# QueensGambit/CrazyAra

Measured on AMD Instinct MI355X. Metric: nn_evals_per_sec, higher is better.
Workload: dtype f16x3; 1 GPU; crazyhouse RISEv2 19-block (34x8x8 planes -> 5184 policy + value), batch=256, inputs resident in HBM, random-init seeded weights; batch=256, parallelism=replicas x1, precision=float16x3

## Files before the change

crazyara_amd/csrc/nn/kernels.h:

```cpp
#pragma once
#include <hip/hip_runtime.h>
#include <cstdint>

namespace cra {

typedef _Float16 half_t;

constexpr int kSquares = 64;

inline int64_t packed_weight_elems(int cout_pad, int k_total) { return int64_t(cout_pad) * k_total; }

struct ConvArgs {
    const void* x;
    const void* wpk;
    const void* wpk_lo;
    const float* bias;
    const void* resid;
    void* out;
    int batch;
    int cin;
    int cout_pad;
    int cout_real;
    int cout_ld;
    int ks;
// ... 237 lines not shown
    int batch, C, cv, fc;
    float* dbg;
    int lds_pad;
    int variant;
};
template <typename T> void prepare_value_head(const ValueHeadArgs& a);
size_t value_head_lds_bytes(const ValueHeadArgs& a);
template <typename T> void launch_value_head(const ValueHeadArgs& a, hipStream_t s);

struct HeadsSmallArgs {
    ConvArgs conv;
    ValueHeadArgs vh;
};
bool heads_small_fits(const ConvArgs& c, const ValueHeadArgs& v);
void launch_heads_small(const HeadsSmallArgs& a, hipStream_t s);

struct ValueFinalArgs {
    const void* in;
    int n;
    const float* w;
    float b[4];
    int wdlp;
    float* value;
    float* aux;
    int batch;
};
template <typename T> void launch_value_final(const ValueFinalArgs& a, hipStream_t s);

void launch_gather_probs(const float* probs, int nb_policy, const uint16_t* idx, const uint32_t* cnt, int stride, int n_slots, float* out,
                         const float* value_dev, float* value_out, int batch, const float* aux_dev, float* aux_out, hipStream_t s);
// ... 23 lines not shown
```

crazyara_amd/csrc/nn/precision.cpp:

```cpp
#include <cstdlib>
#include <stdexcept>

#include "rise_net.h"

namespace cra {

namespace {
constexpr bool kX3ValueHeadOneLaunch = true;
}

RiseNet::DevSwitches::DevSwitches() {
    if (const char* e = getenv("CRA_X3_CONV_DEV")) conv_dev = atoi(e);
    device_graph = getenv("CRA_DEVICE_GRAPH") != nullptr;
    lane_graph = getenv("CRA_LANE_GRAPH") != nullptr;
    lane_no_graph = getenv("CRA_LANE_NO_GRAPH") != nullptr;
    predict_copy = getenv("CRA_PREDICT_COPY") != nullptr;
    predict_zero_copy = getenv("CRA_PREDICT_ZERO_COPY") != nullptr;
    if (const char* e = getenv("CRA_LANE_LAUNCHES")) lane_launches = e[0];
    lane_sync = getenv("CRA_LANE_SYNC") != nullptr;
    if (const char* e = getenv("CRA_X3_TOWER")) x3_symmetric = e[0] == 's';
    if (const char* e = getenv("CRA_X3_SPLIT_DEV")) x3_split_dev = atoi(e);
    no_small_path = getenv("CRA_NO_SMALL_PATH") != nullptr;
    if (const char* e = getenv("CRA_SMALL_BATCH_CONV_SPLIT")) small_conv_split = atoi(e);
    tower_trace = getenv("CRA_TOWER_TRACE") != nullptr;
    x3_value_one_launch = kX3ValueHeadOneLaunch;
    if (const char* e = getenv("CRA_X3_VALUE_HEAD")) x3_value_one_launch = e[0] == 'o';
    value_head_debug = getenv("CRA_VALUE_HEAD_DEBUG") != nullptr;
    if (const char* e = getenv("CRA_VALUE_HEAD_LDS_PAD")) value_head_lds_pad = atoi(e);
    if (const char* e = getenv("CRA_VALUE_HEAD_VARIANT")) value_head_variant = atoi(e);
    x3_no_head_chain = getenv("CRA_X3_NO_HEAD_CHAIN") != nullptr;
    x3_no_tail = getenv("CRA_X3_NO_TAIL") != nullptr;
    small_batch_heads_apart = getenv("CRA_SMALL_BATCH_HEADS_APART") != nullptr;
}

Precision parse_precision(const std::string& precision) {
    Precision v;
    std::string prec = precision;
    auto strip = [&](const std::string& tag) {
        if (prec.size() <= tag.size() || prec.compare(prec.size() - tag.size(), tag.size(), tag) != 0) return false;
        prec.resize(prec.size() - tag.size());
        return true;
    };
    if (strip("-3k")) v.one_launch = false;
    if (strip("-8w")) v.thin_waves = true;
    if (strip("-1wg")) v.board_split = false;
// ... 31 lines not shown
```

crazyara_amd/csrc/nn/rise_net.h:

```cpp
#pragma once
#include <hip/hip_runtime.h>
#include <memory>
#include <string>
#include <utility>
#include <vector>

#include "board_net.h"
#include "netfile.h"

namespace cra {

uint8_t float_to_e4m3(float v);
uint8_t float_to_e5m2(float v);

struct Precision {
    enum class Mode { Float32, Float16, Float16x3, Float16p8, Fp8, Int8 };
    Mode mode = Mode::Float16;
    bool fused = true;
    bool tower = true;
    bool one_launch = true;
    bool thin_waves = false;
    bool board_split = true;
    bool wblock = false;
    bool wnet = false;
// ... 91 lines not shown
        bool lane_no_graph = false;
        bool predict_copy = false;
        bool predict_zero_copy = false;
        char lane_launches = 0;
        bool lane_sync = false;
        bool x3_symmetric = false;
        int x3_split_dev = 0;
        bool no_small_path = false;
        int small_conv_split = 2;
        bool tower_trace = false;
        bool x3_value_one_launch;
        bool value_head_debug = false;
        int value_head_lds_pad = -1;
        int value_head_variant = 0;
        bool x3_no_head_chain = false;
        bool x3_no_tail = false;
        bool small_batch_heads_apart = false;
        DevSwitches();
    } dev_;
    float* value_head_dbg_ = nullptr;

    std::string model_file_path_;
    Precision prec_;
    std::vector<std::pair<float, float>> int8_calib_;
    static constexpr int kBoardSplitMaxBatch = 64;
    std::unique_ptr<RiseNet> small_;
    bool owns_stream_ = true;
    int stream_slot_ = -1;
    std::string precision_arg_;
    int cu_count_ = 256;
// ... 14 lines not shown
```

crazyara_amd/csrc/nn/rise_net.hip:

```cpp
#include "rise_net.h"

#include <cmath>
#include <cstdio>
#include <cstring>
#include <fstream>
#include <algorithm>

#include "net_streams.h"
#include "onnx_import.h"
#include "rise_net_impl.h"
#include "../chess/planes_host.h"

namespace cra {

RiseNet::RiseNet(const std::string& model_path, int device_id, int batch_size, const std::string& precision, const RiseNet* parent)
    : BoardNet(device_id), impl_(new Impl) {
    if (batch_size <= 0) throw std::invalid_argument("batch size must be positive");
    precision_arg_ = precision;
    prec_ = parse_precision(precision);
    design_.batch = batch_size;

    std::string dir, file;
    auto ends_with = [&](const char* ext) { const size_t n = strlen(ext); return model_path.size() > n && model_path.compare(model_path.size() - n, n, ext) == 0; };
    if (ends_with(".cranet") || ends_with(".onnx")) {
// ... 60 lines not shown
    const int B = n > 0 ? n : design_.batch;
    const Op& op = im.ops[i];
    auto boards = [&](ConvArgs c) {
        if (n > 0 && c.batch == design_.batch && !c.out_rows_f32) c.batch = n;
        return c;
    };
    const float* planes = io ? io->planes : d_planes_;
    float* value = io ? io->value : d_value_;
    float* probs = io ? io->probs : d_probs_;
    float* aux = (io && d_aux_) ? (io->aux ? io->aux : d_aux_) : d_aux_;
    switch (op.kind) {
        case OpKind::PlanesToAct:
            launch_planes_to_act<T>(op.x == d_planes_ ? planes : static_cast<const float*>(op.x), static_cast<T*>(op.y), B, op.C, im.cin_pad, s);
            break;
        case OpKind::Conv:
            if (prec_.x3() && dev_.conv_dev >= 0) {
                ConvArgs c = boards(op.conv);
                c.dev = dev_.conv_dev;
                if (op.from_planes) c.planes = planes;
                if (op.fused_softmax) { c.softmax_out = probs; if (!keep_logits_) c.out = nullptr; }
                launch_conv_gemm_x3(c, s);
            } else if (prec_.x3() && op.from_planes) {
                ConvArgs c = boards(op.conv);
                c.planes = planes;
                launch_conv_gemm_x3(c, s);
            } else if (prec_.x3() && op.fused_softmax) {
                ConvArgs c = boards(op.conv);
                c.softmax_out = probs;
                if (!keep_logits_) c.out = nullptr;
                launch_conv_gemm_x3(c, s);
            } else if (prec_.x3()) launch_conv_gemm_x3(boards(op.conv), s);
// ... 623 lines not shown
```

crazyara_amd/csrc/nn/rise_net_build.hip:

```cpp
#include <algorithm>
#include <cmath>
#include <cstring>
#include <type_traits>

#include "../chess/planes_host.h"
#include "pack.h"
#include "rise_net_impl.h"

namespace cra {

namespace {
enum class Family {
    Tower,
    X3Tower,
    X3Split,
    Fused,
    WBlock,
    WSplit,
    Layers,
    Transformer,
    WNtb
};
struct BlockPlan {
    Family family;
// ... 48 lines not shown
    void add_se(Op op, bool consumer_fused);
    void stem();
    void dense_tower();
    void dense_layer_blocks();
    void bottleneck_blocks();
    void transformer_block(size_t i);
    void transformer_block_x3w(const NtbFold& n);
    void flush_tower();
    void flush_x3_run();
    void wsplit_finish();
    void one_launch_head();
    void policy_head();
    void softmax();
    void value_head();
    void merge_heads_small();
    void merge_forward();
};

template <typename T> void RiseNet::Builder<T>::read_model() {
    B = net.design_.batch;
    cin = int(nf.num("nb_input_channels"));
    C = int(nf.num("channels", 256));
    const int cop_init = int(nf.num("channels_operating_init"));
    const int cexp = int(nf.num("channel_expansion"));
    cv = int(nf.num("channels_value_head", 8));
    fc = int(nf.num("value_fc_size", 256));
    cp = int(nf.num("channels_policy_head"));
    wdl = nf.num("use_wdl") != 0 && nf.num("use_plys_to_end") != 0;
    std::vector<std::string> kernels = nf.list("kernels");
    se_types = nf.list("se_types");
// ... 784 lines not shown
    im.ops.push_back(op);
}

template <typename T> void RiseNet::Builder<T>::merge_heads_small() {
    std::vector<Op>& ops = im.ops;
    if (x3_split && ops.size() >= 2 && ops.back().kind == OpKind::ValueHead && ops[ops.size() - 2].kind == OpKind::Conv &&
        ops[ops.size() - 2].fused_softmax && heads_small_fits(ops[ops.size() - 2].conv, ops.back().vh) && !dev.small_batch_heads_apart) {
        Op vh = ops.back();
        ops.pop_back();
        Op& op = ops.back();
        op.kind = OpKind::HeadsSmall;
        op.vh = vh.vh;
    }
}

template <typename T> void RiseNet::Builder<T>::merge_forward() {
    std::vector<Op>& ops = im.ops;
    if (prec.one_launch && ops.size() == 3 && ops[0].kind == OpKind::Stem && ops[1].kind == OpKind::Tower && ops[2].kind == OpKind::Head &&
        ops[1].tw.gate_in == nullptr && ops[1].tw.pool_out == nullptr) {
        Op op;
        op.kind = OpKind::Forward;
        op.st = ops[0].st;
        op.tw = ops[1].tw;
        op.hd = ops[2].hd;
        ops.assign(1, op);
        init_forward_kernel_attributes();
    }
}

template <typename T> void RiseNet::build(const NetFile& nf) {
// ... 6 lines not shown
    if (prec_.wnet && b.wblock_ops == 0 && b.wntb_ops == 0)
        throw std::runtime_error("`-wnet` runs the mobile-bottleneck and transformer blocks of 128 / 192 / 224-channel nets in one launch each: no block of this model qualifies (" +
                                 std::to_string(b.C) + " channels, " + (b.dense_blocks ? "dense residual blocks" : "mobile-bottleneck blocks") +
                                 "); use the precision without the suffix");
    if (prec_.wblock && !prec_.wnet && b.wblock_ops == 0)
        throw std::runtime_error("`-wblock` runs the mobile-bottleneck blocks of 128 / 192 / 224-channel nets in one launch each: no block of this model qualifies (" +
                                 std::to_string(b.C) + " channels, " + (b.dense_blocks ? "dense residual blocks" : "mobile-bottleneck blocks") +
                                 "); use the precision without the suffix");
    if (b.head_ok) {
        b.one_launch_head();
    } else {
        b.policy_head();
        b.softmax();
        b.value_head();
        b.merge_heads_small();
    }
    init_block_kernel_attributes<T>();
    init_x3_kernel_attributes();
    init_x3_wblock_kernel_attributes();
    init_x3_wsplit_kernel_attributes();
    init_x3_wntb_kernel_attributes();
    init_tower_kernel_attributes();
    init_restower_kernel_attributes();
    init_head_kernel_attributes();
    b.merge_forward();
    design_.flops_per_position = 2.0 * b.macs;
    launches_ = int(impl_->ops.size());
}

template void RiseNet::build<half_t>(const NetFile& nf);
template void RiseNet::build<float>(const NetFile& nf);

}
// ... 1 lines not shown
```

crazyara_amd/csrc/nn/rise_net_impl.h:

```cpp
#pragma once
#include <stdexcept>
#include <string>
#include <utility>
#include <vector>

#include "kernels.h"
#include "rise_net.h"

namespace cra {

#define HIP_CHECK(expr)                                                                                      \
    do {                                                                                                     \
        hipError_t _e = (expr);                                                                              \
        if (_e != hipSuccess)                                                                                \
            throw std::runtime_error(std::string("HIP error ") + hipGetErrorString(_e) + " at " #expr);      \
    } while (0)

enum class OpKind { PlanesToAct, Conv, Depthwise, SE, ValueHead, Softmax, Block, ValueFinal, SEGate, Tower, Head, Stem, ResTower, Forward, TowerX3, BlockX3Split, X3SplitFinish, HeadsSmall, Attention, BlockX3W, NtbX3W, BlockX3WSplit, X3WSplitFinish };

struct Op {
    OpKind kind;
    ConvArgs conv{};
    bool from_planes = false;
    bool fused_softmax = false;
    const void* x = nullptr;
    void* y = nullptr;
    const float *w0 = nullptr, *w1 = nullptr, *b0 = nullptr;
    int C = 0, ks = 0, se_kind = 0;
    ValueHeadArgs vh{};
    BlockArgs blk{};
    NtbArgs ntb{};
    ValueFinalArgs vf{};
    TowerArgs tw{};
    HeadArgs hd{};
    ResTowerArgs rt{};
    StemArgs st{};
    X3TowerArgs tx{};
    X3SplitArgs xs{};
// ... 44 lines not shown
```

crazyara_amd/csrc/nn/x3.hip:

```cpp
#include "kernels.h"
#include "device_utils.h"
#include "value_head_body.h"
#include "x3_device.h"

#include <algorithm>
#include <cstdlib>
#include <stdexcept>
#include <type_traits>

#ifndef X3_SGB_VALU
#define X3_SGB_VALU 10
#endif

namespace cra {

namespace {

typedef int i32x4_x3 __attribute__((ext_vector_type(4)));
typedef int i32x8_x3 __attribute__((ext_vector_type(8)));
__device__ __forceinline__ uint32_t x3_high_bytes(uint32_t p01, uint32_t p23) {
    return __builtin_amdgcn_perm(p23, p01, 0x07050301u);
}
__device__ __forceinline__ void split4_b8(const float (&v)[4], half4& hi, uint32_t& h8, uint32_t& l8) {
    uint32_t h[2], l[2];
// ... 9 lines not shown
    else asm volatile("" : "+v"(c) : "v"(a), "v"(b));
}
__device__ __forceinline__ i32x8_x3 x3_cat(const half8& lo16, const half8& hi16) {
    return __builtin_shufflevector(__builtin_bit_cast(i32x4_x3, lo16), __builtin_bit_cast(i32x4_x3, hi16), 0, 1, 2, 3, 4, 5, 6, 7);
}

__device__ __forceinline__ float fmac_shr1(float acc, float x, float w) { return fmaf(w, dpp_mov<DPP_ROW_SHR1>(x), acc); }
__device__ __forceinline__ float fmac_shl1(float acc, float x, float w) { return fmaf(w, dpp_mov<DPP_ROW_SHL1>(x), acc); }

__device__ __forceinline__ void mma_x3(const half8& ah, const half8& al, const half8& bh, const half8& bl, f32x4& c) {
    c = __builtin_amdgcn_mfma_f32_16x16x32_f16(al, bh, c, 0, 0, 0);
    c = __builtin_amdgcn_mfma_f32_16x16x32_f16(ah, bl, c, 0, 0, 0);
    c = __builtin_amdgcn_mfma_f32_16x16x32_f16(ah, bh, c, 0, 0, 0);
}

constexpr int X3_KC = 128;
constexpr int X3_ROWP = X3_KC + 8;

}

template <int MT, int NW>
__device__ __forceinline__ void conv_x3_finish(const ConvArgs& a, f32x4 (&acc)[MT][4], const bool (&active)[MT], char* smem, int b, int co_tile0, float acc_scale) {
    constexpr int NTHR = 64 * NW;
    const int tid = threadIdx.x;
    const int wave = tid >> 6, lane = tid & 63;
    const int l15 = lane & 15, lg = lane >> 4;
    if (a.softmax_out) __syncthreads();
#pragma unroll
    for (int m = 0; m < MT; ++m) {
        if (!active[m]) continue;
        const int co0 = (co_tile0 + m) * 16 + lg * 4;
        float bs[4];
#pragma unroll
        for (int r = 0; r < 4; ++r) bs[r] = a.bias[co0 + r];
#pragma unroll
        for (int t = 0; t < 4; ++t) {
            const int sq = t * 16 + l15;
            float v[4];
#pragma unroll
            for (int r = 0; r < 4; ++r) v[r] = fmaf(acc[m][t][r], acc_scale, bs[r]);
            if (a.relu == 2) {
#pragma unroll
                for (int r = 0; r < 4; ++r) v[r] = fmaxf(v[r], 0.f);
            }
            if (a.resid) {
                float rv[4];
                load4<float>(reinterpret_cast<const float*>(a.resid) + (size_t(b) * kSquares + sq) * a.cout_ld + co0, rv);
#pragma unroll
                for (int r = 0; r < 4; ++r) v[r] += rv[r];
            }
            if (a.relu == 1) {
#pragma unroll
                for (int r = 0; r < 4; ++r) v[r] = fmaxf(v[r], 0.f);
            }
            if (a.out_policy_f32) {
                float* o = reinterpret_cast<float*>(a.out) + size_t(b) * a.cout_real * kSquares;
                float* lds_logits = reinterpret_cast<float*>(smem);
#pragma unroll
                for (int r = 0; r < 4; ++r)
                    if (co0 + r < a.cout_real) {
                        if (a.out) o[(co0 + r) * kSquares + sq] = v[r];
                        if (a.softmax_out) lds_logits[(co0 + r) * kSquares + sq] = v[r];
                    }
            } else if (a.out_rows_f32) {
                const int row = b * kSquares + sq;
                if (row < a.rows_valid) {
                    float* o = reinterpret_cast<float*>(a.out) + size_t(row) * a.cout_real;
#pragma unroll
                    for (int r = 0; r < 4; ++r)
                        if (co0 + r < a.cout_real) o[co0 + r] = v[r];
                }
            } else if (a.out_flat) {
                float* o = reinterpret_cast<float*>(a.out) + size_t(b) * a.flat_pitch;
#pragma unroll
                for (int r = 0; r < 4; ++r)
                    if (co0 + r < a.cout_real) o[(co0 + r) * kSquares + sq] = v[r];
            } else {
                store4<float>(reinterpret_cast<float*>(a.out) + (size_t(b) * kSquares + sq) * a.cout_ld + co0, v);
            }
        }
    }
    if (a.softmax_out) {
        __syncthreads();
        const float* in = reinterpret_cast<const float*>(smem);
        float* red = reinterpret_cast<float*>(smem) + 8192;
        const int n = a.cout_real * kSquares;
        float* out = a.softmax_out + size_t(b) * n;
        float m = -INFINITY;
        for (int i = tid; i < n; i += NTHR) m = fmaxf(m, in[i]);
#pragma unroll
        for (int off = 32; off > 0; off >>= 1) m = fmaxf(m, __shfl_xor(m, off, 64));
        if (lane == 0) red[wave] = m;
        __syncthreads();
        m = red[0];
#pragma unroll
        for (int i = 1; i < NW; ++i) m = fmaxf(m, red[i]);
        float sum = 0.f;
        for (int i = tid; i < n; i += NTHR) sum += expf(in[i] - m);
#pragma unroll
        for (int off = 32; off > 0; off >>= 1) sum += __shfl_xor(sum, off, 64);
        __syncthreads();
        if (lane == 0) red[wave] = sum;
        __syncthreads();
        sum = red[0];
#pragma unroll
        for (int i = 1; i < NW; ++i) sum += red[i];
        const float c = m + logf(sum);
        for (int i = tid; i < n; i += NTHR) out[i] = expf(in[i] - c);
    }
}

template <int KS, int MT, int NW, int NS>
__device__ __forceinline__ void conv_gemm_x3_body(const ConvArgs& a, char* smem, const int bx, const int b) {
    half_t* xh = reinterpret_cast<half_t*>(smem);
    half_t* xl = xh + 65 * X3_ROWP;
    constexpr int ROWP = X3_ROWP, KC = X3_KC, NTHR = 64 * NW;

    const int tid = threadIdx.x;
    const int wave = tid >> 6, lane = tid & 63;
    const int l15 = lane & 15, lg = lane >> 4;
    const int co_tile0 = (bx * NW + wave) * MT;
    bool active[MT];
#pragma unroll
    for (int m = 0; m < MT; ++m) active[m] = (co_tile0 + m) * 16 < a.cout_pad;
    const int x_ld = a.x_ld ? a.x_ld : a.cin;
// ... 390 lines not shown
#pragma unroll
    for (int t = 0; t < 4; ++t) acc2[0][t] = f32x4{0.f, 0.f, 0.f, 0.f};
    ConvP8Window<1> W;
    if (active[0]) conv_p8_prime<1>(W, wph, wp8, 0, nslab_ci);
    __syncthreads();
    if (active[0]) {
#pragma unroll 1
        for (int pass = 0; pass < 2; ++pass) {
            if (pass == 1) conv_p8_prime<1>(W, wph, wp8, KC, nslab_ci);
            conv_p8_pass<1>(W, ConvP8::xh_of(smem, pass), ConvP8::x8_of(smem, pass), wph, wp8, pass * KC, nslab_ci, l15, lg, acc2);
        }
    }
    conv_x3_finish<1, NW>(a, acc2, active, smem, b, wave, a.acc_scale);
}

namespace {
struct ConvX3 {
    static constexpr int KC = X3_KC, ROWP = X3_ROWP, NS = KC / 32, NSTEP = 9 * NS, D = 3;
    static constexpr size_t buf_bytes = size_t(2) * 65 * ROWP * sizeof(half_t);
    static constexpr size_t lds_bytes = 2 * buf_bytes;
    static __device__ __forceinline__ half_t* xh_of(char* smem, int buf) { return reinterpret_cast<half_t*>(smem + buf * buf_bytes); }
    static __device__ __forceinline__ half_t* xl_of(char* smem, int buf) { return xh_of(smem, buf) + 65 * ROWP; }
};
template <int MT> struct ConvX3Window { half8 wh[ConvX3::D][MT], wl[ConvX3::D][MT]; };
template <int MT>
__device__ __forceinline__ void conv_x3_wload(ConvX3Window<MT>& W, const half8* const (&wph)[MT], const half8* const (&wpl)[MT], int kc0, int nslab_ci, int st) {
    const size_t wo = size_t((st / ConvX3::NS) * nslab_ci + (kc0 >> 5) + st % ConvX3::NS) * 64;
#pragma unroll
    for (int m = 0; m < MT; ++m) { W.wh[st % ConvX3::D][m] = wph[m][wo]; W.wl[st % ConvX3::D][m] = wpl[m][wo]; }
}
template <int MT>
__device__ __forceinline__ void conv_x3_prime(ConvX3Window<MT>& W, const half8* const (&wph)[MT], const half8* const (&wpl)[MT], int kc0, int nslab_ci) {
#pragma unroll
    for (int st = 0; st < ConvX3::D; ++st) conv_x3_wload<MT>(W, wph, wpl, kc0, nslab_ci, st);
}
template <int MT>
__device__ __forceinline__ void conv_x3_pass(ConvX3Window<MT>& W, const half_t* xh, const half_t* xl, const half8* const (&wph)[MT],
                                             const half8* const (&wpl)[MT], int kc0, int nslab_ci, int l15, int lg, f32x4 (&acc)[MT][4]) {
    constexpr int ROWP = ConvX3::ROWP, NS = ConvX3::NS, NSTEP = ConvX3::NSTEP, D = ConvX3::D;
    half8 bh[2][4], bl[2][4];
    auto read_frag = [&](int st) {
        const int tap = st / NS, sl = st % NS, dy = tap / 3 - 1, dx = tap % 3 - 1;
#pragma unroll
        for (int t = 0; t < 4; ++t) {
            const int sq = t * 16 + l15;
            const int ny = (sq >> 3) + dy, nx = (sq & 7) + dx;
            const bool ok = (unsigned(ny) < 8u) && (unsigned(nx) < 8u);
            const int off = (ok ? ny * 8 + nx : 64) * ROWP + lg * 8 + sl * 32;
            bh[st & 1][t] = *reinterpret_cast<const half8*>(xh + off);
            bl[st & 1][t] = *reinterpret_cast<const half8*>(xl + off);
        }
    };
    read_frag(0);
#pragma unroll
    for (int st = 0; st < NSTEP; ++st) {
        if (st + 1 < NSTEP) read_frag(st + 1);
        __builtin_amdgcn_sched_barrier(0);
#pragma unroll
        for (int m = 0; m < MT; ++m)
#pragma unroll
            for (int t = 0; t < 4; ++t) acc[m][t] = __builtin_amdgcn_mfma_f32_16x16x32_f16(W.wl[st % D][m], bh[st & 1][t], acc[m][t], 0, 0, 0);
#pragma unroll
        for (int m = 0; m < MT; ++m)
#pragma unroll
            for (int t = 0; t < 4; ++t) acc[m][t] = __builtin_amdgcn_mfma_f32_16x16x32_f16(W.wh[st % D][m], bl[st & 1][t], acc[m][t], 0, 0, 0);
#pragma unroll
        for (int m = 0; m < MT; ++m)
#pragma unroll
            for (int t = 0; t < 4; ++t) acc[m][t] = __builtin_amdgcn_mfma_f32_16x16x32_f16(W.wh[st % D][m], bh[st & 1][t], acc[m][t], 0, 0, 0);
        if (st + D < NSTEP) conv_x3_wload<MT>(W, wph, wpl, kc0, nslab_ci, st + D);
        __builtin_amdgcn_sched_barrier(0);
    }
}
struct ConvX3Stage {
    static constexpr int NV = kSquares * (ConvX3::KC / 8) / 512;
    float pre[NV][8];
    __device__ __forceinline__ void request(const float* xb, int cin, int kc0, int tid) {
#pragma unroll
        for (int j = 0; j < NV; ++j) {
            const int i = tid + j * 512, r = i / (ConvX3::KC / 8), v = i - r * (ConvX3::KC / 8);
            load8<float>(xb + size_t(r) * cin + kc0 + v * 8, pre[j]);
        }
    }
    __device__ __forceinline__ void split_store(half_t* xh, half_t* xl, int tid) {
#pragma unroll
        for (int j = 0; j < NV; ++j) {
            const int i = tid + j * 512, r = i / (ConvX3::KC / 8), v = i - r * (ConvX3::KC / 8);
            half8 h, l;
            split8(pre[j], h, l);
            *reinterpret_cast<half8*>(xh + r * ConvX3::ROWP + v * 8) = h;
            *reinterpret_cast<half8*>(xl + r * ConvX3::ROWP + v * 8) = l;
        }
    }
};
}

__global__ __launch_bounds__(512) void conv3x3_x3_chain_kernel(const ConvArgs a) {
    extern __shared__ __attribute__((aligned(16))) char smem[];
    constexpr int KC = ConvX3::KC, ROWP = ConvX3::ROWP, NW = 8, C = 256;
    const int b = blockIdx.y;
    const int tid = threadIdx.x;
    const int wave = tid >> 6, lane = tid & 63;
    const int l15 = lane & 15, lg = lane >> 4;
    const float* xb = reinterpret_cast<const float*>(a.x) + size_t(b) * kSquares * C;
    constexpr int nslab_ci = C >> 5, nslab = 9 * nslab_ci;
    {
        const half8 *wph[2], *wpl[2];
#pragma unroll
        for (int m = 0; m < 2; ++m) {
            wph[m] = reinterpret_cast<const half8*>(a.pre_wpk) + size_t(wave * 2 + m) * nslab * 64 + lane;
// ... 1357 lines not shown
```

Before: 350,800 evals/s.

## Fuse float16x3 policy chain and value head into one per-board kernel

Adds a heads_x3 kernel that runs, per board, the policy pre-conv, the policy conv with its softmax, and the value head (1x1 conv, FC1, FC2, tanh) in a single launch. The value-head work is placed on waves left idle by the narrow policy conv, and the board input tile staged in LDS is shared by both heads. This removes one kernel launch and a second read of the trunk output. The cost is a larger LDS footprint per workgroup, which may lower occupancy, and a more complex kernel. The shared conv device helpers move into a header so both kernels can use them.

```diff
diff --git a/crazyara_amd/csrc/nn/kernels.h b/crazyara_amd/csrc/nn/kernels.h
--- a/crazyara_amd/csrc/nn/kernels.h
+++ b/crazyara_amd/csrc/nn/kernels.h
@@ -275,6 +275,10 @@
 };
 bool heads_small_fits(const ConvArgs& c, const ValueHeadArgs& v);
 void launch_heads_small(const HeadsSmallArgs& a, hipStream_t s);
+bool heads_x3_fits(const ConvArgs& c, const ValueHeadArgs& v);
+size_t heads_x3_lds_bytes(const ValueHeadArgs& v);
+void launch_heads_x3(const HeadsSmallArgs& a, hipStream_t s);
+void init_x3_heads_kernel_attributes();
 
 struct ValueFinalArgs {
     const void* in;
diff --git a/crazyara_amd/csrc/nn/precision.cpp b/crazyara_amd/csrc/nn/precision.cpp
--- a/crazyara_amd/csrc/nn/precision.cpp
+++ b/crazyara_amd/csrc/nn/precision.cpp
@@ -29,6 +29,7 @@
     if (const char* e = getenv("CRA_VALUE_HEAD_LDS_PAD")) value_head_lds_pad = atoi(e);
     if (const char* e = getenv("CRA_VALUE_HEAD_VARIANT")) value_head_variant = atoi(e);
     x3_no_head_chain = getenv("CRA_X3_NO_HEAD_CHAIN") != nullptr;
+    x3_no_heads_fused = getenv("CRA_X3_NO_HEADS_FUSED") != nullptr;
     x3_no_tail = getenv("CRA_X3_NO_TAIL") != nullptr;
     small_batch_heads_apart = getenv("CRA_SMALL_BATCH_HEADS_APART") != nullptr;
 }
diff --git a/crazyara_amd/csrc/nn/rise_net.h b/crazyara_amd/csrc/nn/rise_net.h
--- a/crazyara_amd/csrc/nn/rise_net.h
+++ b/crazyara_amd/csrc/nn/rise_net.h
@@ -129,6 +129,7 @@
         int value_head_lds_pad = -1;
         int value_head_variant = 0;
         bool x3_no_head_chain = false;
+        bool x3_no_heads_fused = false;
         bool x3_no_tail = false;
         bool small_batch_heads_apart = false;
         DevSwitches();
diff --git a/crazyara_amd/csrc/nn/rise_net.hip b/crazyara_amd/csrc/nn/rise_net.hip
--- a/crazyara_amd/csrc/nn/rise_net.hip
+++ b/crazyara_amd/csrc/nn/rise_net.hip
@@ -98,7 +98,17 @@
             launch_planes_to_act<T>(op.x == d_planes_ ? planes : static_cast<const float*>(op.x), static_cast<T*>(op.y), B, op.C, im.cin_pad, s);
             break;
         case OpKind::Conv:
-            if (prec_.x3() && dev_.conv_dev >= 0) {
+            if (op.heads_fused) {
+                HeadsSmallArgs h;
+                h.conv = boards(op.conv);
+                h.conv.softmax_out = probs;
+                if (!keep_logits_) h.conv.out = nullptr;
+                h.vh = op.vh;
+                h.vh.value = value;
+                h.vh.aux = aux;
+                h.vh.batch = h.conv.batch;
+                launch_heads_x3(h, s);
+            } else if (prec_.x3() && dev_.conv_dev >= 0) {
                 ConvArgs c = boards(op.conv);
                 c.dev = dev_.conv_dev;
                 if (op.from_planes) c.planes = planes;
diff --git a/crazyara_amd/csrc/nn/rise_net_build.hip b/crazyara_amd/csrc/nn/rise_net_build.hip
--- a/crazyara_amd/csrc/nn/rise_net_build.hip
+++ b/crazyara_amd/csrc/nn/rise_net_build.hip
@@ -86,6 +86,7 @@
     void softmax();
     void value_head();
     void merge_heads_small();
+    void merge_heads_x3();
     void merge_forward();
 };
 
@@ -900,6 +901,19 @@
     }
 }
 
+template <typename T> void RiseNet::Builder<T>::merge_heads_x3() {
+    std::vector<Op>& ops = im.ops;
+    if (ops.size() < 2 || ops.back().kind != OpKind::ValueHead || ops[ops.size() - 2].kind != OpKind::Conv) return;
+    const Op& pol = ops[ops.size() - 2];
+    if (!prec.x3() || prec.p8() || !pol.conv.pre_wpk || !pol.fused_softmax || !dev.x3_value_one_launch || dev.x3_no_heads_fused || dev.conv_dev >= 0 ||
+        B <= kBoardSplitMaxBatch || C != 256 || pol.conv.x != ops.back().vh.x || !heads_x3_fits(pol.conv, ops.back().vh))
+        return;
+    Op vh = ops.back();
+    ops.pop_back();
+    ops.back().heads_fused = true;
+    ops.back().vh = vh.vh;
+}
+
 template <typename T> void RiseNet::Builder<T>::merge_forward() {
     std::vector<Op>& ops = im.ops;
     if (prec.one_launch && ops.size() == 3 && ops[0].kind == OpKind::Stem && ops[1].kind == OpKind::Tower && ops[2].kind == OpKind::Head &&
@@ -936,9 +950,11 @@
         b.softmax();
         b.value_head();
         b.merge_heads_small();
+        b.merge_heads_x3();
     }
     init_block_kernel_attributes<T>();
     init_x3_kernel_attributes();
+    init_x3_heads_kernel_attributes();
     init_x3_wblock_kernel_attributes();
     init_x3_wsplit_kernel_attributes();
     init_x3_wntb_kernel_attributes();
diff --git a/crazyara_amd/csrc/nn/rise_net_impl.h b/crazyara_amd/csrc/nn/rise_net_impl.h
--- a/crazyara_amd/csrc/nn/rise_net_impl.h
+++ b/crazyara_amd/csrc/nn/rise_net_impl.h
@@ -22,6 +22,7 @@
     OpKind kind;
     ConvArgs conv{};
     bool from_planes = false;
+    bool heads_fused = false;
     bool fused_softmax = false;
     const void* x = nullptr;
     void* y = nullptr;
diff --git a/crazyara_amd/csrc/nn/x3.hip b/crazyara_amd/csrc/nn/x3.hip
--- a/crazyara_amd/csrc/nn/x3.hip
+++ b/crazyara_amd/csrc/nn/x3.hip
@@ -1,6 +1,7 @@
 #include "kernels.h"
 #include "device_utils.h"
 #include "value_head_body.h"
+#include "x3_conv_device.h"
 #include "x3_device.h"
 
 #include <algorithm>
@@ -47,101 +48,9 @@
     c = __builtin_amdgcn_mfma_f32_16x16x32_f16(ah, bh, c, 0, 0, 0);
 }
 
-constexpr int X3_KC = 128;
-constexpr int X3_ROWP = X3_KC + 8;
-
-}
-
-template <int MT, int NW>
-__device__ __forceinline__ void conv_x3_finish(const ConvArgs& a, f32x4 (&acc)[MT][4], const bool (&active)[MT], char* smem, int b, int co_tile0, float acc_scale) {
-    constexpr int NTHR = 64 * NW;
-    const int tid = threadIdx.x;
-    const int wave = tid >> 6, lane = tid & 63;
-    const int l15 = lane & 15, lg = lane >> 4;
-    if (a.softmax_out) __syncthreads();
-#pragma unroll
-    for (int m = 0; m < MT; ++m) {
-        if (!active[m]) continue;
-        const int co0 = (co_tile0 + m) * 16 + lg * 4;
-        float bs[4];
-#pragma unroll
-        for (int r = 0; r < 4; ++r) bs[r] = a.bias[co0 + r];
-#pragma unroll
-        for (int t = 0; t < 4; ++t) {
-            const int sq = t * 16 + l15;
-            float v[4];
-#pragma unroll
-            for (int r = 0; r < 4; ++r) v[r] = fmaf(acc[m][t][r], acc_scale, bs[r]);
-            if (a.relu == 2) {
-#pragma unroll
-                for (int r = 0; r < 4; ++r) v[r] = fmaxf(v[r], 0.f);
-            }
-            if (a.resid) {
-                float rv[4];
-                load4<float>(reinterpret_cast<const float*>(a.resid) + (size_t(b) * kSquares + sq) * a.cout_ld + co0, rv);
-#pragma unroll
-                for (int r = 0; r < 4; ++r) v[r] += rv[r];
-            }
-            if (a.relu == 1) {
-#pragma unroll
-                for (int r = 0; r < 4; ++r) v[r] = fmaxf(v[r], 0.f);
-            }
-            if (a.out_policy_f32) {
-                float* o = reinterpret_cast<float*>(a.out) + size_t(b) * a.cout_real * kSquares;
-                float* lds_logits = reinterpret_cast<float*>(smem);
-#pragma unroll
-                for (int r = 0; r < 4; ++r)
-                    if (co0 + r < a.cout_real) {
-                        if (a.out) o[(co0 + r) * kSquares + sq] = v[r];
-                        if (a.softmax_out) lds_logits[(co0 + r) * kSquares + sq] = v[r];
-                    }
-            } else if (a.out_rows_f32) {
-                const int row = b * kSquares + sq;
-                if (row < a.rows_valid) {
-                    float* o = reinterpret_cast<float*>(a.out) + size_t(row) * a.cout_real;
-#pragma unroll
-                    for (int r = 0; r < 4; ++r)
-                        if (co0 + r < a.cout_real) o[co0 + r] = v[r];
-                }
-            } else if (a.out_flat) {
-                float* o = reinterpret_cast<float*>(a.out) + size_t(b) * a.flat_pitch;
-#pragma unroll
-                for (int r = 0; r < 4; ++r)
-                    if (co0 + r < a.cout_real) o[(co0 + r) * kSquares + sq] = v[r];
-            } else {
-                store4<float>(reinterpret_cast<float*>(a.out) + (size_t(b) * kSquares + sq) * a.cout_ld + co0, v);
-            }
-        }
-    }
-    if (a.softmax_out) {
-        __syncthreads();
-        const float* in = reinterpret_cast<const float*>(smem);
-        float* red = reinterpret_cast<float*>(smem) + 8192;
-        const int n = a.cout_real * kSquares;
-        float* out = a.softmax_out + size_t(b) * n;
-        float m = -INFINITY;
-        for (int i = tid; i < n; i += NTHR) m = fmaxf(m, in[i]);
-#pragma unroll
-        for (int off = 32; off > 0; off >>= 1) m = fmaxf(m, __shfl_xor(m, off, 64));
-        if (lane == 0) red[wave] = m;
-        __syncthreads();
-        m = red[0];
-#pragma unroll
-        for (int i = 1; i < NW; ++i) m = fmaxf(m, red[i]);
-        float sum = 0.f;
-        for (int i = tid; i < n; i += NTHR) sum += expf(in[i] - m);
-#pragma unroll
-        for (int off = 32; off > 0; off >>= 1) sum += __shfl_xor(sum, off, 64);
-        __syncthreads();
-        if (lane == 0) red[wave] = sum;
-        __syncthreads();
-        sum = red[0];
-#pragma unroll
-        for (int i = 1; i < NW; ++i) sum += red[i];
-        const float c = m + logf(sum);
-        for (int i = tid; i < n; i += NTHR) out[i] = expf(in[i] - c);
-    }
-}
+
+}
+
 
 template <int KS, int MT, int NW, int NS>
 __device__ __forceinline__ void conv_gemm_x3_body(const ConvArgs& a, char* smem, const int bx, const int b) {
@@ -562,86 +471,6 @@
     conv_x3_finish<1, NW>(a, acc2, active, smem, b, wave, a.acc_scale);
 }
 
-namespace {
-struct ConvX3 {
-    static constexpr int KC = X3_KC, ROWP = X3_ROWP, NS = KC / 32, NSTEP = 9 * NS, D = 3;
-    static constexpr size_t buf_bytes = size_t(2) * 65 * ROWP * sizeof(half_t);
-    static constexpr size_t lds_bytes = 2 * buf_bytes;
-    static __device__ __forceinline__ half_t* xh_of(char* smem, int buf) { return reinterpret_cast<half_t*>(smem + buf * buf_bytes); }
-    static __device__ __forceinline__ half_t* xl_of(char* smem, int buf) { return xh_of(smem, buf) + 65 * ROWP; }
-};
-template <int MT> struct ConvX3Window { half8 wh[ConvX3::D][MT], wl[ConvX3::D][MT]; };
-template <int MT>
-__device__ __forceinline__ void conv_x3_wload(ConvX3Window<MT>& W, const half8* const (&wph)[MT], const half8* const (&wpl)[MT], int kc0, int nslab_ci, int st) {
-    const size_t wo = size_t((st / ConvX3::NS) * nslab_ci + (kc0 >> 5) + st % ConvX3::NS) * 64;
-#pragma unroll
-    for (int m = 0; m < MT; ++m) { W.wh[st % ConvX3::D][m] = wph[m][wo]; W.wl[st % ConvX3::D][m] = wpl[m][wo]; }
-}
-template <int MT>
-__device__ __forceinline__ void conv_x3_prime(ConvX3Window<MT>& W, const half8* const (&wph)[MT], const half8* const (&wpl)[MT], int kc0, int nslab_ci) {
-#pragma unroll
-    for (int st = 0; st < ConvX3::D; ++st) conv_x3_wload<MT>(W, wph, wpl, kc0, nslab_ci, st);
-}
-template <int MT>
-__device__ __forceinline__ void conv_x3_pass(ConvX3Window<MT>& W, const half_t* xh, const half_t* xl, const half8* const (&wph)[MT],
-                                             const half8* const (&wpl)[MT], int kc0, int nslab_ci, int l15, int lg, f32x4 (&acc)[MT][4]) {
-    constexpr int ROWP = ConvX3::ROWP, NS = ConvX3::NS, NSTEP = ConvX3::NSTEP, D = ConvX3::D;
-    half8 bh[2][4], bl[2][4];
-    auto read_frag = [&](int st) {
-        const int tap = st / NS, sl = st % NS, dy = tap / 3 - 1, dx = tap % 3 - 1;
-#pragma unroll
-        for (int t = 0; t < 4; ++t) {
-            const int sq = t * 16 + l15;
-            const int ny = (sq >> 3) + dy, nx = (sq & 7) + dx;
-            const bool ok = (unsigned(ny) < 8u) && (unsigned(nx) < 8u);
-            const int off = (ok ? ny * 8 + nx : 64) * ROWP + lg * 8 + sl * 32;
-            bh[st & 1][t] = *reinterpret_cast<const half8*>(xh + off);
-            bl[st & 1][t] = *reinterpret_cast<const half8*>(xl + off);
-        }
-    };
-    read_frag(0);
-#pragma unroll
-    for (int st = 0; st < NSTEP; ++st) {
-        if (st + 1 < NSTEP) read_frag(st + 1);
-        __builtin_amdgcn_sched_barrier(0);
-#pragma unroll
-        for (int m = 0; m < MT; ++m)
-#pragma unroll
-            for (int t = 0; t < 4; ++t) acc[m][t] = __builtin_amdgcn_mfma_f32_16x16x32_f16(W.wl[st % D][m], bh[st & 1][t], acc[m][t], 0, 0, 0);
-#pragma unroll
-        for (int m = 0; m < MT; ++m)
-#pragma unroll
-            for (int t = 0; t < 4; ++t) acc[m][t] = __builtin_amdgcn_mfma_f32_16x16x32_f16(W.wh[st % D][m], bl[st & 1][t], acc[m][t], 0, 0, 0);
-#pragma unroll
-        for (int m = 0; m < MT; ++m)
-#pragma unroll
-            for (int t = 0; t < 4; ++t) acc[m][t] = __builtin_amdgcn_mfma_f32_16x16x32_f16(W.wh[st % D][m], bh[st & 1][t], acc[m][t], 0, 0, 0);
-        if (st + D < NSTEP) conv_x3_wload<MT>(W, wph, wpl, kc0, nslab_ci, st + D);
-        __builtin_amdgcn_sched_barrier(0);
-    }
-}
-struct ConvX3Stage {
-    static constexpr int NV = kSquares * (ConvX3::KC / 8) / 512;
-    float pre[NV][8];
-    __device__ __forceinline__ void request(const float* xb, int cin, int kc0, int tid) {
-#pragma unroll
-        for (int j = 0; j < NV; ++j) {
-            const int i = tid + j * 512, r = i / (ConvX3::KC / 8), v = i - r * (ConvX3::KC / 8);
-            load8<float>(xb + size_t(r) * cin + kc0 + v * 8, pre[j]);
-        }
-    }
-    __device__ __forceinline__ void split_store(half_t* xh, half_t* xl, int tid) {
-#pragma unroll
-        for (int j = 0; j < NV; ++j) {
-            const int i = tid + j * 512, r = i / (ConvX3::KC / 8), v = i - r * (ConvX3::KC / 8);
-            half8 h, l;
-            split8(pre[j], h, l);
-            *reinterpret_cast<half8*>(xh + r * ConvX3::ROWP + v * 8) = h;
-            *reinterpret_cast<half8*>(xl + r * ConvX3::ROWP + v * 8) = l;
-        }
-    }
-};
-}
 
 __global__ __launch_bounds__(512) void conv3x3_x3_chain_kernel(const ConvArgs a) {
     extern __shared__ __attribute__((aligned(16))) char smem[];
diff --git a/crazyara_amd/csrc/nn/x3_conv_device.h b/crazyara_amd/csrc/nn/x3_conv_device.h
--- /dev/null
+++ b/crazyara_amd/csrc/nn/x3_conv_device.h
@@ -0,0 +1,185 @@
+#pragma once
+#include "kernels.h"
+#include "device_utils.h"
+#include "x3_device.h"
+
+namespace cra {
+
+namespace {
+constexpr int X3_KC = 128;
+constexpr int X3_ROWP = X3_KC + 8;
+}
+
+template <int MT, int NW>
+__device__ __forceinline__ void conv_x3_finish(const ConvArgs& a, f32x4 (&acc)[MT][4], const bool (&active)[MT], char* smem, int b, int co_tile0, float acc_scale) {
+    constexpr int NTHR = 64 * NW;
+    const int tid = threadIdx.x;
+    const int wave = tid >> 6, lane = tid & 63;
+    const int l15 = lane & 15, lg = lane >> 4;
+    if (a.softmax_out) __syncthreads();
+#pragma unroll
+    for (int m = 0; m < MT; ++m) {
+        if (!active[m]) continue;
+        const int co0 = (co_tile0 + m) * 16 + lg * 4;
+        float bs[4];
+#pragma unroll
+        for (int r = 0; r < 4; ++r) bs[r] = a.bias[co0 + r];
+#pragma unroll
+        for (int t = 0; t < 4; ++t) {
+            const int sq = t * 16 + l15;
+            float v[4];
+#pragma unroll
+            for (int r = 0; r < 4; ++r) v[r] = fmaf(acc[m][t][r], acc_scale, bs[r]);
+            if (a.relu == 2) {
+#pragma unroll
+                for (int r = 0; r < 4; ++r) v[r] = fmaxf(v[r], 0.f);
+            }
+            if (a.resid) {
+                float rv[4];
+                load4<float>(reinterpret_cast<const float*>(a.resid) + (size_t(b) * kSquares + sq) * a.cout_ld + co0, rv);
+#pragma unroll
+                for (int r = 0; r < 4; ++r) v[r] += rv[r];
+            }
+            if (a.relu == 1) {
+#pragma unroll
+                for (int r = 0; r < 4; ++r) v[r] = fmaxf(v[r], 0.f);
+            }
+            if (a.out_policy_f32) {
+                float* o = reinterpret_cast<float*>(a.out) + size_t(b) * a.cout_real * kSquares;
+                float* lds_logits = reinterpret_cast<float*>(smem);
+#pragma unroll
+                for (int r = 0; r < 4; ++r)
+                    if (co0 + r < a.cout_real) {
+                        if (a.out) o[(co0 + r) * kSquares + sq] = v[r];
+                        if (a.softmax_out) lds_logits[(co0 + r) * kSquares + sq] = v[r];
+                    }
+            } else if (a.out_rows_f32) {
+                const int row = b * kSquares + sq;
+                if (row < a.rows_valid) {
+                    float* o = reinterpret_cast<float*>(a.out) + size_t(row) * a.cout_real;
+#pragma unroll
+                    for (int r = 0; r < 4; ++r)
+                        if (co0 + r < a.cout_real) o[co0 + r] = v[r];
+                }
+            } else if (a.out_flat) {
+                float* o = reinterpret_cast<float*>(a.out) + size_t(b) * a.flat_pitch;
+#pragma unroll
+                for (int r = 0; r < 4; ++r)
+                    if (co0 + r < a.cout_real) o[(co0 + r) * kSquares + sq] = v[r];
+            } else {
+                store4<float>(reinterpret_cast<float*>(a.out) + (size_t(b) * kSquares + sq) * a.cout_ld + co0, v);
+            }
+        }
+    }
+    if (a.softmax_out) {
+        __syncthreads();
+        const float* in = reinterpret_cast<const float*>(smem);
+        float* red = reinterpret_cast<float*>(smem) + 8192;
+        const int n = a.cout_real * kSquares;
+        float* out = a.softmax_out + size_t(b) * n;
+        float m = -INFINITY;
+        for (int i = tid; i < n; i += NTHR) m = fmaxf(m, in[i]);
+#pragma unroll
+        for (int off = 32; off > 0; off >>= 1) m = fmaxf(m, __shfl_xor(m, off, 64));
+        if (lane == 0) red[wave] = m;
+        __syncthreads();
+        m = red[0];
+#pragma unroll
+        for (int i = 1; i < NW; ++i) m = fmaxf(m, red[i]);
+        float sum = 0.f;
+        for (int i = tid; i < n; i += NTHR) sum += expf(in[i] - m);
+#pragma unroll
+        for (int off = 32; off > 0; off >>= 1) sum += __shfl_xor(sum, off, 64);
+        __syncthreads();
+        if (lane == 0) red[wave] = sum;
+        __syncthreads();
+        sum = red[0];
+#pragma unroll
+        for (int i = 1; i < NW; ++i) sum += red[i];
+        const float c = m + logf(sum);
+        for (int i = tid; i < n; i += NTHR) out[i] = expf(in[i] - c);
+    }
+}
+
+namespace {
+struct ConvX3 {
+    static constexpr int KC = X3_KC, ROWP = X3_ROWP, NS = KC / 32, NSTEP = 9 * NS, D = 3;
+    static constexpr size_t buf_bytes = size_t(2) * 65 * ROWP * sizeof(half_t);
+    static constexpr size_t lds_bytes = 2 * buf_bytes;
+    static __device__ __forceinline__ half_t* xh_of(char* smem, int buf) { return reinterpret_cast<half_t*>(smem + buf * buf_bytes); }
+    static __device__ __forceinline__ half_t* xl_of(char* smem, int buf) { return xh_of(smem, buf) + 65 * ROWP; }
+};
+template <int MT> struct ConvX3Window { half8 wh[ConvX3::D][MT], wl[ConvX3::D][MT]; };
+template <int MT>
+__device__ __forceinline__ void conv_x3_wload(ConvX3Window<MT>& W, const half8* const (&wph)[MT], const half8* const (&wpl)[MT], int kc0, int nslab_ci, int st) {
+    const size_t wo = size_t((st / ConvX3::NS) * nslab_ci + (kc0 >> 5) + st % ConvX3::NS) * 64;
+#pragma unroll
+    for (int m = 0; m < MT; ++m) { W.wh[st % ConvX3::D][m] = wph[m][wo]; W.wl[st % ConvX3::D][m] = wpl[m][wo]; }
+}
+template <int MT>
+__device__ __forceinline__ void conv_x3_prime(ConvX3Window<MT>& W, const half8* const (&wph)[MT], const half8* const (&wpl)[MT], int kc0, int nslab_ci) {
+#pragma unroll
+    for (int st = 0; st < ConvX3::D; ++st) conv_x3_wload<MT>(W, wph, wpl, kc0, nslab_ci, st);
+}
+template <int MT>
+__device__ __forceinline__ void conv_x3_pass(ConvX3Window<MT>& W, const half_t* xh, const half_t* xl, const half8* const (&wph)[MT],
+                                             const half8* const (&wpl)[MT], int kc0, int nslab_ci, int l15, int lg, f32x4 (&acc)[MT][4]) {
+    constexpr int ROWP = ConvX3::ROWP, NS = ConvX3::NS, NSTEP = ConvX3::NSTEP, D = ConvX3::D;
+    half8 bh[2][4], bl[2][4];
+    auto read_frag = [&](int st) {
+        const int tap = st / NS, sl = st % NS, dy = tap / 3 - 1, dx = tap % 3 - 1;
+#pragma unroll
+        for (int t = 0; t < 4; ++t) {
+            const int sq = t * 16 + l15;
+            const int ny = (sq >> 3) + dy, nx = (sq & 7) + dx;
+            const bool ok = (unsigned(ny) < 8u) && (unsigned(nx) < 8u);
+            const int off = (ok ? ny * 8 + nx : 64) * ROWP + lg * 8 + sl * 32;
+            bh[st & 1][t] = *reinterpret_cast<const half8*>(xh + off);
+            bl[st & 1][t] = *reinterpret_cast<const half8*>(xl + off);
+        }
+    };
+    read_frag(0);
+#pragma unroll
+    for (int st = 0; st < NSTEP; ++st) {
+        if (st + 1 < NSTEP) read_frag(st + 1);
+        __builtin_amdgcn_sched_barrier(0);
+#pragma unroll
+        for (int m = 0; m < MT; ++m)
+#pragma unroll
+            for (int t = 0; t < 4; ++t) acc[m][t] = __builtin_amdgcn_mfma_f32_16x16x32_f16(W.wl[st % D][m], bh[st & 1][t], acc[m][t], 0, 0, 0);
+#pragma unroll
+        for (int m = 0; m < MT; ++m)
+#pragma unroll
+            for (int t = 0; t < 4; ++t) acc[m][t] = __builtin_amdgcn_mfma_f32_16x16x32_f16(W.wh[st % D][m], bl[st & 1][t], acc[m][t], 0, 0, 0);
+#pragma unroll
+        for (int m = 0; m < MT; ++m)
+#pragma unroll
+            for (int t = 0; t < 4; ++t) acc[m][t] = __builtin_amdgcn_mfma_f32_16x16x32_f16(W.wh[st % D][m], bh[st & 1][t], acc[m][t], 0, 0, 0);
+        if (st + D < NSTEP) conv_x3_wload<MT>(W, wph, wpl, kc0, nslab_ci, st + D);
+        __builtin_amdgcn_sched_barrier(0);
+    }
+}
+struct ConvX3Stage {
+    static constexpr int NV = kSquares * (ConvX3::KC / 8) / 512;
+    float pre[NV][8];
+    __device__ __forceinline__ void request(const float* xb, int cin, int kc0, int tid) {
+#pragma unroll
+        for (int j = 0; j < NV; ++j) {
+            const int i = tid + j * 512, r = i / (ConvX3::KC / 8), v = i - r * (ConvX3::KC / 8);
+            load8<float>(xb + size_t(r) * cin + kc0 + v * 8, pre[j]);
+        }
+    }
+    __device__ __forceinline__ void split_store(half_t* xh, half_t* xl, int tid) {
+#pragma unroll
+        for (int j = 0; j < NV; ++j) {
+            const int i = tid + j * 512, r = i / (ConvX3::KC / 8), v = i - r * (ConvX3::KC / 8);
+            half8 h, l;
+            split8(pre[j], h, l);
+            *reinterpret_cast<half8*>(xh + r * ConvX3::ROWP + v * 8) = h;
+            *reinterpret_cast<half8*>(xl + r * ConvX3::ROWP + v * 8) = l;
+        }
+    }
+};
+}
+
+}
diff --git a/crazyara_amd/csrc/nn/x3_heads.cpp b/crazyara_amd/csrc/nn/x3_heads.cpp
--- /dev/null
+++ b/crazyara_amd/csrc/nn/x3_heads.cpp
@@ -0,0 +1,222 @@
+#include "x3_conv_device.h"
+#include "value_head_body.h"
+
+#include <stdexcept>
+
+namespace cra {
+
+namespace {
+struct HeadsX3 {
+    static constexpr int C = 256, XP = C + 4;
+    static constexpr size_t xs_off = ConvX3::lds_bytes;
+    static constexpr size_t xs_bytes = size_t(kSquares) * XP * sizeof(float);
+    static constexpr int RB = 8, NBUF = 4;
+    static size_t lds_bytes(int cv) { return xs_off + xs_bytes + (size_t(cv) * C + size_t(kSquares) * cv + 8) * sizeof(float); }
+    static_assert(xs_off % 16 == 0 && xs_bytes % 16 == 0, "16-byte rows");
+};
+
+__device__ __forceinline__ void heads_x3_store_f32(const ConvX3Stage& st, float* xs, int kc0, int tid) {
+#pragma unroll
+    for (int j = 0; j < ConvX3Stage::NV; ++j) {
+        const int i = tid + j * 512, r = i / (ConvX3::KC / 8), v = i - r * (ConvX3::KC / 8);
+        float* p = xs + r * HeadsX3::XP + kc0 + v * 8;
+        *reinterpret_cast<f32x4*>(p) = f32x4{st.pre[j][0], st.pre[j][1], st.pre[j][2], st.pre[j][3]};
+        *reinterpret_cast<f32x4*>(p + 4) = f32x4{st.pre[j][4], st.pre[j][5], st.pre[j][6], st.pre[j][7]};
+    }
+}
+
+__device__ __forceinline__ void heads_x3_fc1(const ValueHeadArgs& v, const float* s_flat, float* s_part, int kq0, int kq1, int lane) {
+    constexpr int RB = HeadsX3::RB, NBUF = HeadsX3::NBUF;
+    const int nq = kSquares * v.cv / 8, nrow = (kq1 - kq0) * nq;
+    for (int j4 = lane; 4 * j4 < v.fc; j4 += 64) {
+        const float* wt = v.w1t + size_t(kq0) * nq * v.fc + 4 * j4;
+        const float* fl = s_flat + kq0 * nq;
+        f32x4 w[NBUF][RB];
+        auto request = [&](int u, int row) {
+#pragma unroll
+            for (int j = 0; j < RB; ++j) w[u][j] = *reinterpret_cast<const f32x4*>(wt + size_t(row + j) * v.fc);
+        };
+#pragma unroll
+        for (int u = 0; u < NBUF; ++u) request(u, u * RB);
+        f32x4 h = {0.f, 0.f, 0.f, 0.f};
+        int kq = kq0;
+#pragma unroll 1
+        for (int i = 0; i < nrow; i += NBUF * RB) {
+#pragma unroll
+            for (int u = 0; u < NBUF; ++u) {
+#pragma unroll
+                for (int q = 0; q < RB / 4; ++q) {
+                    const f32x4 f = *reinterpret_cast<const f32x4*>(fl + i + u * RB + 4 * q);
+#pragma unroll
+                    for (int e = 0; e < 4; ++e) {
+                        float h0 = h[0], h1 = h[1], h2 = h[2], h3 = h[3];
+                        const float w0 = w[u][4 * q + e][0], w1 = w[u][4 * q + e][1], w2 = w[u][4 * q + e][2], w3 = w[u][4 * q + e][3], fe = f[e];
+                        asm volatile("v_fmac_f32 %0, %4, %8\n\tv_fmac_f32 %1, %5, %8\n\tv_fmac_f32 %2, %6, %8\n\tv_fmac_f32 %3, %7, %8"
+                                     : "+v"(h0), "+v"(h1), "+v"(h2), "+v"(h3) : "v"(w0), "v"(w1), "v"(w2), "v"(w3), "v"(fe));
+                        h = f32x4{h0, h1, h2, h3};
+                    }
+                }
+                if (i + (NBUF + u) * RB < nrow) request(u, i + (NBUF + u) * RB);
+            }
+            if ((i + NBUF * RB) % nq == 0) {
+                *reinterpret_cast<f32x4*>(s_part + kq * v.fc + 4 * j4) = h;
+                h = f32x4{0.f, 0.f, 0.f, 0.f};
+                ++kq;
+            }
+        }
+    }
+}
+}
+
+__global__ __launch_bounds__(512) void heads_x3_kernel(const HeadsSmallArgs args) {
+    extern __shared__ __attribute__((aligned(16))) char smem[];
+    const ConvArgs& a = args.conv;
+    const ValueHeadArgs& vh = args.vh;
+    constexpr int KC = ConvX3::KC, ROWP = ConvX3::ROWP, NW = 8, C = HeadsX3::C, XP = HeadsX3::XP;
+    const int b = blockIdx.y;
+    const int tid = threadIdx.x;
+    const int wave = __builtin_amdgcn_readfirstlane(tid >> 6), lane = tid & 63;
+    const int l15 = lane & 15, lg = lane >> 4;
+    const float* xb = reinterpret_cast<const float*>(a.x) + size_t(b) * kSquares * C;
+    constexpr int nslab_ci = C >> 5, nslab = 9 * nslab_ci;
+    float* xs = reinterpret_cast<float*>(smem + HeadsX3::xs_off);
+    float* ws = xs + kSquares * XP;
+    float* s_flat = ws + vh.cv * C;
+    float* s_red = s_flat + kSquares * vh.cv;
+    {
+        const half8 *wph[2], *wpl[2];
+#pragma unroll
+        for (int m = 0; m < 2; ++m) {
+            wph[m] = reinterpret_cast<const half8*>(a.pre_wpk) + size_t(wave * 2 + m) * nslab * 64 + lane;
+            wpl[m] = reinterpret_cast<const half8*>(a.pre_wpk_lo) + size_t(wave * 2 + m) * nslab * 64 + lane;
+        }
+        f32x4 acc[2][4];
+#pragma unroll
+        for (int m = 0; m < 2; ++m)
+#pragma unroll
+            for (int t = 0; t < 4; ++t) acc[m][t] = f32x4{0.f, 0.f, 0.f, 0.f};
+        for (int i = tid; i < 4 * ROWP; i += 512) {
+            const int tile = i / ROWP, c = i - tile * ROWP;
+            (tile & 1 ? ConvX3::xl_of(smem, tile >> 1) : ConvX3::xh_of(smem, tile >> 1))[64 * ROWP + c] = half_t(0.f);
+        }
+        const int nwc = vh.cv * C;
+        f32x4 wv[2];
+#pragma unroll
+        for (int u = 0; u < 2; ++u)
+            if (tid * 4 + u * 2048 < nwc) wv[u] = *reinterpret_cast<const f32x4*>(vh.wconv + tid * 4 + u * 2048);
+        ConvX3Stage stage;
+        stage.request(xb, C, 0, tid);
+        stage.split_store(ConvX3::xh_of(smem, 0), ConvX3::xl_of(smem, 0), tid);
+        heads_x3_store_f32(stage, xs, 0, tid);
+#pragma unroll
+        for (int u = 0; u < 2; ++u)
+            if (tid * 4 + u * 2048 < nwc) *reinterpret_cast<f32x4*>(ws + tid * 4 + u * 2048) = wv[u];
+#pragma unroll 1
+        for (int pass = 0; pass < 2; ++pass) {
+            const int kc0 = pass * KC;
+            ConvX3Window<2> W;
+            conv_x3_prime<2>(W, wph, wpl, kc0, nslab_ci);
+            __syncthreads();
+            if (pass == 0) stage.request(xb, C, KC, tid);
+            conv_x3_pass<2>(W, ConvX3::xh_of(smem, pass), ConvX3::xl_of(smem, pass), wph, wpl, kc0, nslab_ci, l15, lg, acc);
+            if (pass == 0) {
+                stage.split_store(ConvX3::xh_of(smem, 1), ConvX3::xl_of(smem, 1), tid);
+                heads_x3_store_f32(stage, xs, KC, tid);
+            }
+        }
+        __syncthreads();
+#pragma unroll
+        for (int m = 0; m < 2; ++m) {
+            const int c0 = (wave * 2 + m) * 16 + lg * 4;
+            const f32x4 bs = *reinterpret_cast<const f32x4*>(a.pre_bias + c0);
+            half_t* xh = ConvX3::xh_of(smem, c0 >> 7);
+            half_t* xl = ConvX3::xl_of(smem, c0 >> 7);
+#pragma unroll
+            for (int t = 0; t < 4; ++t) {
+                const int sq = t * 16 + l15;
+                float v[4];
+#pragma unroll
+                for (int r = 0; r < 4; ++r) v[r] = fmaxf(fmaf(acc[m][t][r], 1.f, bs[r]), 0.f);
+                half4 h, l;
+                split4(v, h, l);
+                *reinterpret_cast<half4*>(xh + sq * ROWP + (c0 & 127)) = h;
+                *reinterpret_cast<half4*>(xl + sq * ROWP + (c0 & 127)) = l;
+            }
+        }
+    }
+    {
+        const int sq = tid & 63;
+        float acc[2] = {0.f, 0.f};
+        const float* xr = xs + sq * XP;
+        for (int c = 0; c < C; c += 4) {
+            const f32x4 xv = *reinterpret_cast<const f32x4*>(xr + c);
+#pragma unroll
+            for (int k = 0; k < 2; ++k) {
+                const int co = wave + NW * k;
+                if (co < vh.cv) {
+                    const f32x4 wv = *reinterpret_cast<const f32x4*>(ws + co * C + c);
+                    acc[k] = fmaf(wv[0], xv[0], acc[k]);
+                    acc[k] = fmaf(wv[1], xv[1], acc[k]);
+                    acc[k] = fmaf(wv[2], xv[2], acc[k]);
+                    acc[k] = fmaf(wv[3], xv[3], acc[k]);
+                }
+            }
+        }
+#pragma unroll
+        for (int k = 0; k < 2; ++k) {
+            const int co = wave + NW * k;
+            if (co < vh.cv) s_flat[co * kSquares + sq] = fmaxf(acc[k] + vh.bconv[co], 0.f);
+        }
+    }
+    const int ntile = a.cout_pad >> 4;
+    bool active[1] = {wave < ntile};
+    const half8 *wph[1], *wpl[1];
+    wph[0] = reinterpret_cast<const half8*>(a.wpk) + size_t(active[0] ? wave : 0) * nslab * 64 + lane;
+    wpl[0] = reinterpret_cast<const half8*>(a.wpk_lo) + size_t(active[0] ? wave : 0) * nslab * 64 + lane;
+    f32x4 acc2[1][4];
+#pragma unroll
+    for (int t = 0; t < 4; ++t) acc2[0][t] = f32x4{0.f, 0.f, 0.f, 0.f};
+    ConvX3Window<1> W;
+    if (active[0]) conv_x3_prime<1>(W, wph, wpl, 0, nslab_ci);
+    __syncthreads();
+    if (active[0]) {
+#pragma unroll 1
+        for (int pass = 0; pass < 2; ++pass) {
+            if (pass == 1) conv_x3_prime<1>(W, wph, wpl, KC, nslab_ci);
+            conv_x3_pass<1>(W, ConvX3::xh_of(smem, pass), ConvX3::xl_of(smem, pass), wph, wpl, pass * KC, nslab_ci, l15, lg, acc2);
+        }
+    } else {
+        const int nidle = NW - ntile, iw = wave - ntile;
+        heads_x3_fc1(vh, s_flat, xs, iw * 8 / nidle, (iw + 1) * 8 / nidle, lane);
+    }
+    conv_x3_finish<1, NW>(a, acc2, active, smem, b, wave, 1.f);
+    const float* s_part = xs;
+    float part = 0.f;
+    for (int t = tid; t < vh.fc; t += 512) {
+        float ps = (s_part[t] + s_part[vh.fc + t]) + (s_part[2 * vh.fc + t] + s_part[3 * vh.fc + t]);
+        ps += (s_part[4 * vh.fc + t] + s_part[5 * vh.fc + t]) + (s_part[6 * vh.fc + t] + s_part[7 * vh.fc + t]);
+        const float h = vh.b1[t] + ps;
+        part = fmaf(vh.w2[t], fmaxf(h, 0.f), part);
+    }
+    const float tot = block_sum<512>(part, s_red);
+    if (tid == 0) vh.value[b] = tanhf(tot + vh.b2);
+}
+
+bool heads_x3_fits(const ConvArgs& c, const ValueHeadArgs& v) {
+    return c.pre_wpk && !c.p8 && c.ks == 3 && c.cin == 256 && c.cout_pad <= 96 && !c.resid && !c.planes && !c.out_rows_f32 && c.out_policy_f32 &&
+           c.cout_real * kSquares <= 8192 && !v.dbg && v.lds_pad < 0 && v.variant == 0 && !v.wwdl && v.w1t && v.C == 256 && v.cv >= 1 && v.cv <= 16 &&
+           v.cv % 4 == 0 && v.fc % 4 == 0 && size_t(8) * v.fc * sizeof(float) <= HeadsX3::xs_bytes && HeadsX3::lds_bytes(v.cv) <= 160 * 1024;
+}
+size_t heads_x3_lds_bytes(const ValueHeadArgs& v) { return HeadsX3::lds_bytes(v.cv); }
+
+void init_x3_heads_kernel_attributes() {
+    (void)hipFuncSetAttribute(reinterpret_cast<const void*>(&heads_x3_kernel), hipFuncAttributeMaxDynamicSharedMemorySize, 160 * 1024);
+}
+
+void launch_heads_x3(const HeadsSmallArgs& a, hipStream_t s) {
+    if (!heads_x3_fits(a.conv, a.vh) || !a.conv.softmax_out || a.conv.batch != a.vh.batch || a.conv.x != a.vh.x)
+        throw std::invalid_argument("heads_x3_kernel: the float16x3 policy chain (256 -> 256 -> at most 96 couts, with its softmax) and the one-launch FC value head of the same boards");
+    hipLaunchKernelGGL(heads_x3_kernel, dim3(1, a.conv.batch), dim3(512), HeadsX3::lds_bytes(a.vh.cv), s, a);
+}
+
+}
```

Measured after the change: 353,300 evals/s, median of 5. No clear change (+0.7%).
